# sleep3r/crispy

Measured on AMD Instinct MI355X. Metric: concurrent real-time 48 kHz streams/GPU (RNNoise), higher is better.
Workload: dtype f32; 1 GPU; Batched RNNoise: 4096 concurrent 48 kHz mono streams per GPU x 100 frames per step (BASELINE configs[1]), seeded synthetic int8 weights; streams_per_gpu=4096, output_finite=True

## Files before the change

### crispy_amd/csrc/crispy_api.cpp

```cpp
#include "../../include/crispy_hip.h"
#include "api_util.h"
#include "rn_common.h"
#include "rn_handle.h"

#include <cmath>
#include <cstdarg>
#include <cstddef>
#include <cstdio>
#include <cstdlib>
#include <cstring>
#include <new>
#include <atomic>
#include <stdexcept>
#include <string>
#include <thread>
#include <vector>

using namespace crispy;

namespace {

constexpr int kChunkFrames = 250;
#ifndef RN_SUB_FRAMES
#define RN_SUB_FRAMES 12
#endif
constexpr int kSubFrames = RN_SUB_FRAMES;
constexpr int kStagedMaxStreams = 1280;

inline const std::vector<int>& ramp_frames() {
  static const std::vector<int> ramp = [] {
    std::vector<int> r;
    if (const char* env = dev_env("CRISPY_RN_RAMP")) {
      for (const char* p = env; *p;) {
        char* end = nullptr;
        const long v = std::strtol(p, &end, 10);
        if (end == p) break;
        if (v > 0) r.push_back(v > kSubFrames ? kSubFrames : (int)v);
        p = *end ? end + 1 : end;
      }
    }
    if (r.empty()) r = {3, 4, 5, 7, 10};
    return r;
  }();
  return ramp;
}
inline int sub_frames(int index, int remaining) {
  const std::vector<int>& ramp = ramp_frames();
  const int want = index < (int)ramp.size() ? ramp[index] : kSubFrames;
  return remaining < want ? remaining : want;
}
inline int count_subs(int T) {
  int n = 0;
  for (int done = 0; done < T; ++n) done += sub_frames(n, T - done);
  return n;
}

void build_tables(RnTables* t) {
  const double pi = 3.14159265358979323846;
  for (int i = 0; i < RN_FRAME; ++i) {
    const double s = std::sin(.5 * pi * (i + .5) / RN_FRAME);
    t->half_window[i] = (float)std::sin(.5 * pi * s * s);
  }
  for (int i = 0; i < RN_NB; ++i)
    for (int j = 0; j < RN_NB; ++j) {
      double v = std::cos((i + .5) * j * pi / RN_NB);
      if (j == 0) v *= std::sqrt(.5);
      t->dct[i * RN_NB + j] = (float)v;
    }
  for (int i = 0; i < 208; ++i)
    t->tansig[i] = i <= 200 ? (float)(std::floor(std::tanh(0.04 * i) * 1e6 + 0.5) / 1e6) : 1.f;
  for (int k = 0; k < RN_WINDOW; ++k) {
    t->w960[k].x = (float)std::cos(-2.0 * pi * k / RN_WINDOW);
    t->w960[k].y = (float)std::sin(-2.0 * pi * k / RN_WINDOW);
  }
  static const int eband[RN_NB] = {0, 1, 2, 3, 4, 5, 6, 7, 8, 10, 12, 14, 16, 20, 24, 28, 34, 40, 48, 60, 78, 100};
  for (int i = 0; i < 24; ++i) t->eband[i] = i < RN_NB ? eband[i] : 100;
  for (int i = 0; i < RN_NB - 1; ++i) {
    const int bs = (eband[i + 1] - eband[i]) * 4;
    for (int j = 0; j < bs; ++j) {
      t->bin_band[eband[i] * 4 + j] = i;
      t->bin_frac[eband[i] * 4 + j] = (float)j / (float)bs;
    }
  }
  {
    int piece[64] = {0}, head[2][RN_NB];
    for (int b = 0; b < RN_NB; ++b) head[0][b] = head[1][b] = 0;
    int lane = 1;
    for (int side = 0; side < 2; ++side)
      for (int b = 0; b < RN_NB; ++b) {
        const int c0 = side == 0 ? (b > 0 ? eband[b - 1] : 0) : eband[b];
        const int c1 = side == 0 ? eband[b] : (b < RN_NB - 1 ? eband[b + 1] : eband[b]);
        const int w = (side == 0 && b == 0) ? 0 : c1 - c0;
        if (w <= 0) continue;
        const int np = (w + 5) / 6;
        if ((lane & 15) + np > 16) lane = (lane + 15) & ~15;
        if (np > 4 || lane + np > 64) std::abort();
        head[side][b] = lane;
        for (int p = 0, c = c0; p < np; ++p) {
          const int n = (w - (c - c0) + (np - p) - 1) / (np - p);
          piece[lane + p] = c | (n << 7) | (side << 10) | ((p + 1 < np ? 1 : 0) << 11) | ((p == 0 && np > 2 ? 1 : 0) << 12);
          c += n;
        }
        lane += np;
      }
    for (int l = 0; l < 64; ++l) {
      const int b = l < RN_NB ? l : 0;
      t->band_piece[l] = piece[l] | (head[0][b] << 13) | (head[1][b] << 19);
    }
  }
}

void pack_matrix(uint32_t* dst, const int8_t* src, int K, int rows, int stride) {
  const int k8n = (K + 7) / 8;
  uint16_t* h = reinterpret_cast<uint16_t*>(dst);
  for (int k8 = 0; k8 < k8n; ++k8)
    for (int r = 0; r < rows; ++r)
      for (int q = 0; q < 8; ++q) {
        const int k = 8 * k8 + q;
        const _Float16 v = (_Float16)(float)(k < K ? src[(size_t)k * stride + r] : 0);
        uint16_t bits;
        std::memcpy(&bits, &v, 2);
        h[((size_t)k8 * rows + r) * 8 + q] = bits;
      }
}

void pack_matrix8(uint32_t* dst, const int8_t* src, int K, int rows, int stride) {
  const int k16n = (K + 15) / 16;
  int8_t* b = reinterpret_cast<int8_t*>(dst);
  for (int k16 = 0; k16 < k16n; ++k16)
    for (int r = 0; r < rows; ++r)
      for (int q = 0; q < 16; ++q) {
        const int k = 16 * k16 + q;
        b[((size_t)k16 * rows + r) * 16 + q] = k < K ? src[(size_t)k * stride + r] : 0;
      }
}

void pack_bias(uint32_t* dst, const int8_t* src, int n) {
  for (int i = 0; i < n; ++i) {
    const float f = (float)src[i];
    std::memcpy(&dst[i], &f, 4);
  }
}

void pack_weights(std::vector<uint32_t>& out, const int8_t* w) {
  out.assign(RnPack8::END, 0);
  uint32_t* p = out.data();
  pack_matrix(p + 4 * RnPack::ID_W, w + RnBlob::ID_W, 42, 24, 24);
  pack_matrix(p + 4 * RnPack::VG_W, w + RnBlob::VG_W, 24, 72, 72);
  pack_matrix(p + 4 * RnPack::VG_R, w + RnBlob::VG_R, 24, 72, 72);
  pack_matrix(p + 4 * RnPack::VO_W, w + RnBlob::VO_W, 24, 1, 1);
  pack_matrix(p + 4 * RnPack::NG_W, w + RnBlob::NG_W, 90, 144, 144);
  pack_matrix(p + 4 * RnPack::NG_R, w + RnBlob::NG_R, 48, 144, 144);
  pack_matrix(p + 4 * RnPack::DG_W, w + RnBlob::DG_W, 114, 288, 288);
  pack_matrix(p + 4 * RnPack::DG_R, w + RnBlob::DG_R, 96, 288, 288);
  pack_matrix(p + 4 * RnPack::DO_W, w + RnBlob::DO_W, 96, 22, 22);
  pack_bias(p + RnPack::ID_B, w + RnBlob::ID_B, 24);
  pack_bias(p + RnPack::VG_B, w + RnBlob::VG_B, 72);
  pack_bias(p + RnPack::VO_B, w + RnBlob::VO_B, 1);
  pack_bias(p + RnPack::NG_B, w + RnBlob::NG_B, 144);
  pack_bias(p + RnPack::DG_B, w + RnBlob::DG_B, 288);
  pack_bias(p + RnPack::DO_B, w + RnBlob::DO_B, 22);
  pack_matrix8(p + 4 * RnPack8::ID_W, w + RnBlob::ID_W, 42, 24, 24);
// ... 602 lines not shown
```

### crispy_amd/csrc/rn_common.h

```cpp
#pragma once
#include <hip/hip_runtime.h>
#include <stdint.h>

namespace crispy {

constexpr int RN_FRAME = 480;
constexpr int RN_WINDOW = 960;
constexpr int RN_NFREQ = 481;
constexpr int RN_NB = 22;
constexpr int RN_NFEAT = 42;
constexpr int RN_PITCH_BUF = 1728;
constexpr int RN_HIST = 1920;
constexpr int RN_HIST_FRAMES = 4;
constexpr int RN_TAPS = 72;
constexpr int RN_WEIGHT_BYTES = 87503;
constexpr int RN_DBG_FLOATS = 4304;

struct RnTables {
  float half_window[RN_FRAME];
  float dct[RN_NB * RN_NB];
  float tansig[208];
  float2 w960[RN_WINDOW];
  float bin_frac[400];
  int bin_band[400];
  int eband[24];
  int band_piece[64];
};

struct RnBlob {
  static constexpr int ID_W = 0, ID_B = ID_W + 42 * 24;
  static constexpr int VG_W = ID_B + 24, VG_R = VG_W + 24 * 72, VG_B = VG_R + 24 * 72;
  static constexpr int VO_W = VG_B + 72, VO_B = VO_W + 24;
  static constexpr int NG_W = VO_B + 1, NG_R = NG_W + 90 * 144, NG_B = NG_R + 48 * 144;
  static constexpr int DG_W = NG_B + 144, DG_R = DG_W + 114 * 288, DG_B = DG_R + 96 * 288;
  static constexpr int DO_W = DG_B + 288, DO_B = DO_W + 96 * 22;
  static constexpr int END = DO_B + 22;
};
static_assert(RnBlob::END == RN_WEIGHT_BYTES, "blob layout");

constexpr int rn_k8(int k) { return (k + 7) / 8; }
struct RnPack {
  static constexpr int ID_W = 0;
  static constexpr int VG_W = ID_W + rn_k8(42) * 24;
  static constexpr int VG_R = VG_W + rn_k8(24) * 72;
  static constexpr int VO_W = VG_R + rn_k8(24) * 72;
  static constexpr int NG_W = VO_W + rn_k8(24) * 1;
  static constexpr int NG_R = NG_W + rn_k8(90) * 144;
  static constexpr int DG_W = NG_R + rn_k8(48) * 144;
  static constexpr int DG_R = DG_W + rn_k8(114) * 288;
  static constexpr int DO_W = DG_R + rn_k8(96) * 288;
  static constexpr int MAT_END = DO_W + rn_k8(96) * 22;
  static constexpr int ID_B = MAT_END * 4;
  static constexpr int VG_B = ID_B + 24;
  static constexpr int VO_B = VG_B + 72;
  static constexpr int NG_B = VO_B + 1;
  static constexpr int DG_B = NG_B + 144;
  static constexpr int DO_B = DG_B + 288;
  static constexpr int END = DO_B + 22;
};

constexpr int rn_k16(int k) { return (k + 15) / 16; }
struct RnPack8 {
  static constexpr int ID_W = (RnPack::END + 3) / 4;
  static constexpr int VG_W = ID_W + rn_k16(42) * 24;
  static constexpr int VG_R = VG_W + rn_k16(24) * 72;
  static constexpr int NG_W = VG_R + rn_k16(24) * 72;
  static constexpr int NG_R = NG_W + rn_k16(90) * 144;
  static constexpr int DG_W = NG_R + rn_k16(48) * 144;
  static constexpr int DG_R = DG_W + rn_k16(114) * 288;
  static constexpr int DO_W = DG_R + rn_k16(96) * 288;
  static constexpr int MAT_END = DO_W + rn_k16(96) * 22;
  static constexpr int END = MAT_END * 4;
};

struct RnArgs {
  const float* in;
  float* out;
  long stride_t, stride_b;
  int in_s16, out_s16;
// ... 226 lines not shown
```

### crispy_amd/csrc/rn_kernels.hip

```cpp
#include <type_traits>
#include "rn_common.h"
#include "rn_prio.h"
#include "rn_scale.h"
#include "rn_wave_sums.h"

namespace crispy {
namespace {

constexpr int WAVE = 64;

#ifdef RN_PROFILE
#define RN_PROF_DECL long long tprev_ = clock64(); \
  float* profp_ = (DBG && a.dbg) ? a.dbg + (long)blockIdx.x * RN_DBG_FLOATS + 3824 : nullptr; \
  rn_prof_mark(profp_, 14);
#define RN_PROF_LEAVE rn_prof_mark(profp_, 15);
#define STAMP(k) { const long long tn_ = clock64(); if (profp_ && threadIdx.x == 0) profp_[k] += (float)(tn_ - tprev_); tprev_ = tn_; }
__device__ __forceinline__ void rn_prof_mark(float* p, int k) {
  if (p && threadIdx.x == 0) {
    unsigned* u = reinterpret_cast<unsigned*>(p);
    unsigned hw, xcc;
    asm volatile("s_getreg_b32 %0, hwreg(HW_REG_HW_ID)" : "=s"(hw));
    asm volatile("s_getreg_b32 %0, hwreg(HW_REG_XCC_ID)" : "=s"(xcc));
    u[k] = (unsigned)__builtin_amdgcn_s_memrealtime();
    u[k + 2] = (unsigned)__builtin_amdgcn_s_memtime();
    u[18] = hw;
    u[19] = xcc;
  }
}
#elif defined(RN_STOP_AFTER)
#define RN_PROF_DECL
#define RN_PROF_LEAVE
#define STAMP(k) { if ((k) == RN_STOP_AFTER) { __syncthreads(); continue; } }
#else
#define RN_PROF_DECL
#define RN_PROF_LEAVE
#define STAMP(k)
#endif

__device__ __constant__ int c_second_check[16] = {0, 0, 3, 2, 3, 2, 5, 2, 3, 2, 3, 2, 5, 2, 3, 2};

__device__ __forceinline__ float2 cmul(float2 a, float2 b) {
  return make_float2(a.x * b.x - a.y * b.y, a.x * b.y + a.y * b.x);
}
__device__ __forceinline__ float2 cadd(float2 a, float2 b) { return make_float2(a.x + b.x, a.y + b.y); }
__device__ __forceinline__ float2 csub(float2 a, float2 b) { return make_float2(a.x - b.x, a.y - b.y); }
__device__ __forceinline__ float2 cconj(float2 a) { return make_float2(a.x, -a.y); }

template <int CTRL, int ROW_MASK = 0xf>
__device__ __forceinline__ float dpp_mov(float v) {
  const int iv = __float_as_int(v);
  return __int_as_float(__builtin_amdgcn_update_dpp(0, iv, CTRL, ROW_MASK, 0xf, false));
}
template <int CTRL>
__device__ __forceinline__ float dpp_add(float v) {
  float r = v + dpp_mov<CTRL>(v);
  asm volatile("" : "+v"(r));
  return r;
}
template <class V>
__device__ __forceinline__ void lane_put(V& v, V s, int l) {
  static_assert(sizeof(V) == 4, "one dword");
  asm("v_writelane_b32 %0, %1, %2" : "+v"(v) : "s"(s), "n"(l));
}
template <class T>
__device__ __forceinline__ T ld_u32(const T* __restrict__ base, unsigned idx) {
  return *reinterpret_cast<const T*>(reinterpret_cast<const char*>(base) + idx * (unsigned)sizeof(T));
}
__device__ __forceinline__ float wave_sum(float v) {
  v += dpp_mov<0xB1>(v);
  v += dpp_mov<0x4E>(v);
  v += dpp_mov<0x141>(v);
  v += dpp_mov<0x140>(v);
  v += dpp_mov<0x142, 0xa>(v);
  v += dpp_mov<0x143, 0xc>(v);
  return __int_as_float(__builtin_amdgcn_readlane(__float_as_int(v), 63));
}

template <int NW>
__device__ __forceinline__ void rn_sync() {
  if constexpr (NW == 1) {
    __syncthreads();
  } else {
    __builtin_amdgcn_fence(__ATOMIC_RELEASE, "wavefront");
    __builtin_amdgcn_s_waitcnt(0xc07f);
    __builtin_amdgcn_wave_barrier();
    __builtin_amdgcn_fence(__ATOMIC_ACQUIRE, "wavefront");
  }
}

template <int R>
__device__ __forceinline__ void butterfly(const float2 (&v)[R], float2 (&o)[R]);

template <>
__device__ __forceinline__ void butterfly<4>(const float2 (&v)[4], float2 (&o)[4]) {
  const float2 s0 = cadd(v[0], v[2]), d0 = csub(v[0], v[2]);
  const float2 s1 = cadd(v[1], v[3]), d1 = csub(v[1], v[3]);
  o[0] = cadd(s0, s1);
  o[2] = csub(s0, s1);
  o[1] = make_float2(d0.x + d1.y, d0.y - d1.x);
  o[3] = make_float2(d0.x - d1.y, d0.y + d1.x);
}
template <>
__device__ __forceinline__ void butterfly<3>(const float2 (&v)[3], float2 (&o)[3]) {
  const float2 t = cadd(v[1], v[2]), d = csub(v[1], v[2]);
  o[0] = cadd(v[0], t);
  const float2 a = make_float2(v[0].x - 0.5f * t.x, v[0].y - 0.5f * t.y);
  const float s = 0.86602540378443864676f;
  const float2 b = make_float2(s * d.x, s * d.y);
  o[1] = make_float2(a.x + b.y, a.y - b.x);
  o[2] = make_float2(a.x - b.y, a.y + b.x);
}
template <>
__device__ __forceinline__ void butterfly<5>(const float2 (&v)[5], float2 (&o)[5]) {
  const float c1 = 0.30901699437494742410f, s1 = 0.95105651629515357212f;
  const float c2 = -0.80901699437494742410f, s2 = 0.58778525229247312917f;
  const float2 t1 = cadd(v[1], v[4]), t2 = cadd(v[2], v[3]);
  const float2 t3 = csub(v[1], v[4]), t4 = csub(v[2], v[3]);
  o[0] = make_float2(v[0].x + t1.x + t2.x, v[0].y + t1.y + t2.y);
  const float2 a1 = make_float2(v[0].x + c1 * t1.x + c2 * t2.x, v[0].y + c1 * t1.y + c2 * t2.y);
  const float2 a2 = make_float2(v[0].x + c2 * t1.x + c1 * t2.x, v[0].y + c2 * t1.y + c1 * t2.y);
  const float2 b1 = make_float2(s1 * t3.x + s2 * t4.x, s1 * t3.y + s2 * t4.y);
  const float2 b2 = make_float2(s2 * t3.x - s1 * t4.x, s2 * t3.y - s1 * t4.y);
  o[1] = make_float2(a1.x + b1.y, a1.y - b1.x);
  o[4] = make_float2(a1.x - b1.y, a1.y + b1.x);
  o[2] = make_float2(a2.x + b2.y, a2.y - b2.x);
  o[3] = make_float2(a2.x - b2.y, a2.y + b2.x);
}

template <>
__device__ __forceinline__ void butterfly<8>(const float2 (&v)[8], float2 (&o)[8]) {
  const float2 ev[4] = {v[0], v[2], v[4], v[6]}, od[4] = {v[1], v[3], v[5], v[7]};
  float2 e[4], d[4];
  butterfly<4>(ev, e);
  butterfly<4>(od, d);
  const float h = 0.70710678118654752f;
  const float2 t0 = d[0];
  const float2 t1 = make_float2((d[1].x + d[1].y) * h, (d[1].y - d[1].x) * h);
  const float2 t2 = make_float2(d[2].y, -d[2].x);
  const float2 t3 = make_float2((d[3].y - d[3].x) * h, -(d[3].x + d[3].y) * h);
  o[0] = cadd(e[0], t0); o[4] = csub(e[0], t0);
  o[1] = cadd(e[1], t1); o[5] = csub(e[1], t1);
  o[2] = cadd(e[2], t2); o[6] = csub(e[2], t2);
  o[3] = cadd(e[3], t3); o[7] = csub(e[3], t3);
}

#define RN_VGPR_CAP __attribute__((amdgpu_num_vgpr(60)))
template <int R, int NS>
__device__ __forceinline__ int fft_rd(int j, int r) {
  constexpr int M = 480 / R;
  if (R == 8 && NS == 4) return (j & 3) * 120 + (j >> 2) + 15 * r;
  if (R == 3 && NS == 32) {
    const int i = j + r * M;
    return i ^ (((i >> 5) & 3) << 2);
  }
  return j + r * M;
}
template <int R, int NS>
__device__ __forceinline__ int fft_wr(int j, int r) {
  if (R == 4 && NS == 1) return r * 120 + j;
  if (R == 8 && NS == 4) {
    const int a = j >> 2, m = j & 3;
    return 32 * a + m + 4 * (r ^ (a & 3));
  }
  const int k = j % NS;
  return (j / NS) * NS * R + k + r * NS;
}
template <int NW, int R, int NS, int NSIG>
__device__ __forceinline__ void fft_pass_n(float2* const (&bufs)[NSIG], const float2* __restrict__ w960, int lane) {
  constexpr int M = 480 / R;
  constexpr int NBF = (M + WAVE - 1) / WAVE;
  float2 o[NSIG][NBF][R];
  constexpr int NTW = (NS > 1 && WAVE % NS == 0) ? 1 : NBF;
  float2 tw[NTW][R];
  if (NS > 1) {
#pragma unroll
    for (int nb = 0; nb < NTW; ++nb) {
      const unsigned k = (unsigned)min(lane + WAVE * nb, M - 1) % NS;
#pragma unroll
      for (int r = 1; r < R; ++r) tw[nb][r] = ld_u32(w960, k * (unsigned)(r * (960 / (NS * R))));
    }
  }
#pragma unroll
  for (int nb = 0; nb < NBF; ++nb) {
    const int j = lane + WAVE * nb;
    if (j < M) {
#pragma unroll
      for (int g = 0; g < NSIG; ++g) {
        float2 v[R];
#pragma unroll
        for (int r = 0; r < R; ++r) {
          float2 x = bufs[g][fft_rd<R, NS>(j, r)];
          if (NS > 1 && r > 0) x = cmul(x, tw[NTW == 1 ? 0 : nb][r]);
          v[r] = x;
        }
        butterfly<R>(v, o[g][nb]);
      }
    }
  }
  rn_sync<NW>();
#pragma unroll
  for (int nb = 0; nb < NBF; ++nb) {
    const int j = lane + WAVE * nb;
    if (j < M) {
#pragma unroll
      for (int g = 0; g < NSIG; ++g) {
#pragma unroll
        for (int r = 0; r < R; ++r) bufs[g][fft_wr<R, NS>(j, r)] = o[g][nb][r];
      }
    }
  }
  rn_sync<NW>();
}
template <int NW, int R, int NS>
__device__ __forceinline__ void fft_pass(float2* buf, const float2* __restrict__ w960, int lane) {
  float2* const bufs[1] = {buf};
  fft_pass_n<NW, R, NS, 1>(bufs, w960, lane);
}

template <int NW>
__device__ __forceinline__ void fft480(float2* buf, const float2* __restrict__ w960, int lane) {
  fft_pass<NW, 4, 1>(buf, w960, lane);
  fft_pass<NW, 8, 4>(buf, w960, lane);
  fft_pass<NW, 3, 32>(buf, w960, lane);
  fft_pass<NW, 5, 96>(buf, w960, lane);
}

template <int NW, int NSIG, class In>
__device__ __forceinline__ void fft480_from(float2* const (&bufs)[NSIG], In in, const float2* __restrict__ w960, int lane) {
  {
    float2 o[NSIG][2][4];
#pragma unroll
    for (int nb = 0; nb < 2; ++nb) {
      const int j = lane + WAVE * nb;
      if (j < 120) {
#pragma unroll
        for (int g = 0; g < NSIG; ++g) {
          float2 v[4];
#pragma unroll
          for (int r = 0; r < 4; ++r) v[r] = in(g, j, r);
          butterfly<4>(v, o[g][nb]);
        }
      }
    }
#pragma unroll
    for (int nb = 0; nb < 2; ++nb) {
      const int j = lane + WAVE * nb;
      if (j < 120) {
#pragma unroll
        for (int g = 0; g < NSIG; ++g) {
#pragma unroll
          for (int r = 0; r < 4; ++r) bufs[g][fft_wr<4, 1>(j, r)] = o[g][nb][r];
        }
      }
    }
    rn_sync<NW>();
  }
  fft_pass_n<NW, 8, 4, NSIG>(bufs, w960, lane);
  fft_pass_n<NW, 3, 32, NSIG>(bufs, w960, lane);
  fft_pass_n<NW, 5, 96, NSIG>(bufs, w960, lane);
}

template <int NW, int NSIG>
__device__ __forceinline__ void real_fwd_post(float2* const (&bufs)[NSIG], const float2* __restrict__ w960, int lane) {
  const float scale = 1.0f / 960.0f;
  float2 wk[4], wn[4];
#pragma unroll
  for (int m = 0; m < 4; ++m) {
    const unsigned k = (unsigned)min(lane + WAVE * m, 240);
    wk[m] = ld_u32(w960, k);
    wn[m] = ld_u32(w960, 480u - k);
  }
#pragma unroll
  for (int m = 0; m < 4; ++m) {
    const int k = lane + WAVE * m;
    if (k <= 240) {
#pragma unroll
      for (int g = 0; g < NSIG; ++g) {
        float2* buf = bufs[g];
        const float2 zk = buf[k];
        const float2 zn = (k == 0) ? zk : buf[480 - k];
        float2 zc = cconj(zn);
        float2 fe = make_float2(0.5f * (zk.x + zc.x), 0.5f * (zk.y + zc.y));
        float2 d = make_float2(0.5f * (zk.x - zc.x), 0.5f * (zk.y - zc.y));
        float2 t = cmul(wk[m], make_float2(d.y, -d.x));
        const float2 xk = make_float2((fe.x + t.x) * scale, (fe.y + t.y) * scale);
        zc = cconj(zk);
        fe = make_float2(0.5f * (zn.x + zc.x), 0.5f * (zn.y + zc.y));
        d = make_float2(0.5f * (zn.x - zc.x), 0.5f * (zn.y - zc.y));
        t = cmul(wn[m], make_float2(d.y, -d.x));
        const float2 xn = make_float2((fe.x + t.x) * scale, (fe.y + t.y) * scale);
        buf[k] = xk;
        buf[480 - k] = xn;
      }
    }
  }
  rn_sync<NW>();
}

template <int NW>
__device__ __forceinline__ void real_inv_pre(float2* buf, const float2* __restrict__ w960, int lane) {
  float2 wk[4], wn[4];
#pragma unroll
  for (int m = 0; m < 4; ++m) {
    const unsigned k = (unsigned)min(lane + WAVE * m, 240);
    wk[m] = ld_u32(w960, k);
    wn[m] = ld_u32(w960, 480u - k);
  }
#pragma unroll
  for (int m = 0; m < 4; ++m) {
    const int k = lane + WAVE * m;
    if (k <= 240) {
      const float2 a = buf[k];
      const float2 bn = buf[480 - k];
      float2 b = cconj(bn);
      float2 fe = cadd(a, b);
      float2 fo = cmul(csub(a, b), cconj(wk[m]));
      const float2 zk = make_float2(fe.x - fo.y, -(fe.y + fo.x));
      b = cconj(a);
      fe = cadd(bn, b);
      fo = cmul(csub(bn, b), cconj(wn[m]));
      const float2 zn = make_float2(fe.x - fo.y, -(fe.y + fo.x));
      buf[k] = zk;
      if (k > 0) buf[480 - k] = zn;
    }
  }
  rn_sync<NW>();
}

struct BandEdges {
  int piece;
};

__device__ __forceinline__ float band_sum(const float* part_lo, const float* part_hi, const BandEdges& be, int lane) {
  int bd = be.piece;
  asm volatile("" : "+v"(bd));
  const int n = (bd >> 7) & 7;
  const float* p = ((bd >> 10) & 1 ? part_lo : part_hi) + (bd & 127);
  float v[6];
#pragma unroll
  for (int k = 0; k < 6; ++k) v[k] = p[k];
  float s = 0.f;
#pragma unroll
  for (int k = 0; k < 6; ++k) s += k < n ? v[k] : 0.f;
  {
    const float t1 = dpp_mov<0x101>(s);
    s += (bd >> 11) & 1 ? t1 : 0.f;
    const float t2 = dpp_mov<0x102>(s);
    s += (bd >> 12) & 1 ? t2 : 0.f;
  }
  const float rise = __int_as_float(__builtin_amdgcn_ds_bpermute(((bd >> 13) & 63) << 2, __float_as_int(s)));
  const float fall = __int_as_float(__builtin_amdgcn_ds_bpermute(((bd >> 19) & 63) << 2, __float_as_int(s)));
  float tot = rise + fall;
  if (lane == 0 || lane == RN_NB - 1) tot *= 2.f;
  return tot;
}

template <int NW, bool CORR, bool XE = false>
__device__ __forceinline__ void band_pairs(const float2* S, const float2* Xc, float* part, float* Eout, float* Cout,
                                           float* Xout, float2* park, const RnTables* __restrict__ tab,
                                           const BandEdges& be, int lane) {
  float clo[4], chi[4];
  float xlo[4], xhi[4];
  float2 fr[4];
#pragma unroll
  for (int m = 0; m < 4; ++m) fr[m] = ld_u32(reinterpret_cast<const float2*>(tab->bin_frac), (unsigned)min(lane + WAVE * m, 199));
  float4 svq[4];
#pragma unroll
  for (int m = 0; m < 4; ++m) svq[m] = *reinterpret_cast<const float4*>(S + 2 * min(lane + WAVE * m, 199));
#pragma unroll
  for (int m = 0; m < 4; ++m) {
    const int pidx = lane + WAVE * m;
    clo[m] = 0.f; chi[m] = 0.f;
    if (pidx < 200) {
      const float2 f = fr[m];
      const float4 sv = svq[m];
      float e0 = sv.x * sv.x; e0 += sv.y * sv.y;
      float e1 = sv.z * sv.z; e1 += sv.w * sv.w;
      float lo = (1.f - f.x) * e0 + (1.f - f.y) * e1;
      float hi = f.x * e0 + f.y * e1;
      lo = dpp_add<0xB1>(lo);
      hi = dpp_add<0xB1>(hi);
      if ((lane & 1) == 0) { part[pidx >> 1] = lo; part[100 + (pidx >> 1)] = hi; }
      if (CORR) {
        const float4 xv = *reinterpret_cast<const float4*>(Xc + 2 * pidx);
        float c0 = xv.x * sv.x; c0 += xv.y * sv.y;
        float c1 = xv.z * sv.z; c1 += xv.w * sv.w;
        float l2 = (1.f - f.x) * c0 + (1.f - f.y) * c1;
        float h2 = f.x * c0 + f.y * c1;
        clo[m] = dpp_add<0xB1>(l2);
        chi[m] = dpp_add<0xB1>(h2);
        if (XE) {
          float x0, x1, l3, h3;
          if (m == 0) {
            x0 = fmaf(xv.y, xv.y, xv.x * xv.x);
            x1 = fmaf(xv.w, xv.w, xv.z * xv.z);
            l3 = fmaf(1.f - f.y, x1, (1.f - f.x) * x0);
            h3 = fmaf(f.y, x1, f.x * x0);
          } else {
            x0 = fmaf(xv.x, xv.x, xv.y * xv.y);
            x1 = fmaf(xv.z, xv.z, xv.w * xv.w);
            l3 = fmaf(1.f - f.x, x0, (1.f - f.y) * x1);
// ... 232 lines not shown
                                            float* state, float* zbuf, signed char* st_img, int toff,
                                            const TansigTab& tansig, int lane) {
  constexpr int ROWS = 3 * N;
  constexpr int MK16 = (M + 15) / 16, NK16 = (N + 15) / 16;
  constexpr int NRZ = (2 * N + WAVE - 1) / WAVE, NRC = (N + WAVE - 1) / WAVE;
  const float S = 1.f / 256.f;
  const RnScale sst = image_i8<NK16 * 16>(st_img, lane, [&](int i) { return i < N ? state[min(i, N - 1)] : 0.f; });
  rn_sync<NW>();
  {
    int rows[NRZ];
    float acc[NRZ];
#pragma unroll
    for (int r = 0; r < NRZ; ++r) {
      rows[r] = min(lane + WAVE * r, 2 * N - 1);
      acc[r] = ld_u32(bias, (unsigned)rows[r]);
    }
    dotn_i<MK16, NK16, ROWS, NRZ, rn_chains(NW)>(rs, w_off, u_off, rows, in_img, st_img, toff, sin, sst.dn, acc);
#pragma unroll
    for (int r = 0; r < NRZ; ++r) {
      const int row = lane + WAVE * r;
      const float s = sigmoid_approx(S * acc[r], tansig);
      if (row < 2 * N) {
        if (row < N) zbuf[row] = s;
        else digits_store(st_img, row - N, state[row - N] * s, sst.up);
      }
    }
  }
  rn_sync<NW>();
  {
    int rows[NRC];
    float acc[NRC];
#pragma unroll
    for (int r = 0; r < NRC; ++r) {
      rows[r] = 2 * N + min(lane + WAVE * r, N - 1);
      acc[r] = ld_u32(bias, (unsigned)rows[r]);
    }
    dotn_i<MK16, NK16, ROWS, NRC, rn_chains(NW)>(rs, w_off, u_off, rows, in_img, st_img, toff, sin, sst.dn, acc);
#pragma unroll
    for (int r = 0; r < NRC; ++r) {
      const int i = lane + WAVE * r;
      if (i < N) {
        float c = S * acc[r];
        c = c < 0.f ? 0.f : c;
        const float z = zbuf[i];
        state[i] = z * state[i] + (1.f - z) * c;
      }
    }
  }
  rn_sync<NW>();
}

struct alignas(16) RnSlot {
  float2 A[482];
  float2 Bb[482];
  float U[200];
  float Ex[24], Ep[24], Exp[24];
  int pitch_index;
  float pitch_gain;
  int silence;
  int pad;
};
template <int NW> struct RnLdsT;
template <> struct alignas(16) RnLdsT<1> {
  RnSlot s[1];
  float ceps[8 * 22];
  float rnn_state[168];
};
template <> struct alignas(16) RnLdsT<3> {
  RnSlot s[2];
  float2 pa[482];
  float2 pb[482];
  float ceps[8 * 22];
  float rnn_state[168];
  int pitch_index[2];
  float pitch_gain[2];
};
static_assert(sizeof(RnLdsT<1>) <= 10240, "16 workgroups per CU need <= 10 KB of LDS each");
static_assert(6 * sizeof(RnLdsT<3>) <= 160 * 1024, "six stage-pipelined streams per CU");

constexpr int U_G = 0, U_R = 24, U_VAD = 46, U_LY = 48;
constexpr int PL_FEAT = 800, PL_Z = 842, PL_DENSE = 938, PL_A_FREE = 800, PL_U_FREE = 48;

__device__ __forceinline__ float lane_up(float v, int lane4, int off) {
  return __int_as_float(__builtin_amdgcn_ds_bpermute(lane4 + 4 * (WAVE - off), __float_as_int(v)));
}

struct Cand {
  float num, den;
  int idx;
};
__device__ __forceinline__ bool cand_better(const Cand& a, const Cand& b) {
  const float l = a.num * b.den, r = b.num * a.den;
  const bool gt = l > r, ngt = !(r > l), lt = a.idx < b.idx;
  return gt | (ngt & lt);
}
__device__ __forceinline__ Cand cand_pick(bool take_a, const Cand& a, const Cand& b) {
  return Cand{take_a ? a.num : b.num, take_a ? a.den : b.den, take_a ? a.idx : b.idx};
}
template <int OFF>
__device__ __forceinline__ int lane_xor(int v) {
  return __builtin_amdgcn_ds_swizzle(v, (OFF << 10) | 0x1f);
}
template <int OFF>
__device__ __forceinline__ Cand cand_xor(const Cand& c) {
  return Cand{__int_as_float(lane_xor<OFF>(__float_as_int(c.num))), __int_as_float(lane_xor<OFF>(__float_as_int(c.den))),
              lane_xor<OFF>(c.idx)};
}
__device__ __forceinline__ Cand wave_best(Cand c, int half_addr) {
  {
    const Cand o = {__int_as_float(__builtin_amdgcn_ds_bpermute(half_addr, __float_as_int(c.num))),
                    __int_as_float(__builtin_amdgcn_ds_bpermute(half_addr, __float_as_int(c.den))),
                    __builtin_amdgcn_ds_bpermute(half_addr, c.idx)};
    c = cand_pick(cand_better(o, c), o, c);
  }
  { const Cand o = cand_xor<16>(c); c = cand_pick(cand_better(o, c), o, c); }
  { const Cand o = cand_xor<8>(c); c = cand_pick(cand_better(o, c), o, c); }
  { const Cand o = cand_xor<4>(c); c = cand_pick(cand_better(o, c), o, c); }
  { const Cand o = cand_xor<2>(c); c = cand_pick(cand_better(o, c), o, c); }
  { const Cand o = cand_xor<1>(c); c = cand_pick(cand_better(o, c), o, c); }
  c.num = __int_as_float(__builtin_amdgcn_readlane(__float_as_int(c.num), 0));
  c.den = __int_as_float(__builtin_amdgcn_readlane(__float_as_int(c.den), 0));
  c.idx = __builtin_amdgcn_readlane(c.idx, 0);
  return c;
}

typedef float rn_f2 __attribute__((ext_vector_type(2)));
__device__ __forceinline__ void lag_window(const float* xr, int lane, float (&xv)[8]) {
#pragma unroll
  for (int m = 0; m < 7; ++m) xv[m] = xr[WAVE * m];
  xv[7] = 0.f;
  if (lane < 32) xv[7] = xr[WAVE * 7];
// ... 457 lines not shown
          const float g1 = xyk / sqrtf(1.f + xx * yyk);
          float cont;
          if (abs(T1 - prev_period) <= 1) cont = last_gain;
          else if (abs(T1 - prev_period) <= 2 && 5 * k * k < T0) cont = .5f * last_gain;
          else cont = 0.f;
          float thresh = fmaxf(.3f, .7f * g0 - cont);
          if (T1 < 90) thresh = fmaxf(.4f, .85f * g0 - cont);
          else if (T1 < 60) thresh = fmaxf(.5f, .9f * g0 - cont);
          const unsigned long long pass = __ballot(lane < 14 && T1 >= 30 && g1 > thresh);
          if (pass != 0ull) {
            const int w = 63 - __builtin_clzll(pass);
            best_xy = __int_as_float(__builtin_amdgcn_readlane(__float_as_int(xyk), w));
            best_yy = __int_as_float(__builtin_amdgcn_readlane(__float_as_int(yyk), w));
            T = __builtin_amdgcn_readlane(T1, w);
            g = __int_as_float(__builtin_amdgcn_readlane(__float_as_int(g1), w));
          }
        }
        best_xy = fmaxf(0.f, best_xy);
        float pgv = (best_yy <= best_xy) ? 1.f : best_xy / (best_yy + 1.f);
        float xc3[3];
        {
          const float* yr[3] = {x - (T - 1) + lane, x - T + lane, x - (T + 1) + lane};
          float sb[3];
          lag_dots<3, false>(xwin, yr, lane, xc3, sb);
        }
        int offset = 0;
        if ((xc3[2] - xc3[0]) > .7f * (xc3[1] - xc3[0])) offset = 1;
        else if ((xc3[0] - xc3[2]) > .7f * (xc3[1] - xc3[2])) offset = -1;
        if (pgv > g) pgv = g;
        pitch_index = 2 * T + offset;
        if (pitch_index < 60) pitch_index = 60;
        pitch_gain = pgv;
        last_period = pitch_index;
        last_gain = pgv;
      }
      rn_sync<NW>();
      STAMP(4)
      if constexpr (NW > 1) {
        if (lane == 0) { L.pitch_index[t & 1] = pitch_index; L.pitch_gain[t & 1] = pitch_gain; }
      }
    }
    if (own_b) {
      if constexpr (NW > 1) {
        pitch_index = __builtin_amdgcn_readfirstlane(L.pitch_index[t & 1]);
        pitch_gain = L.pitch_gain[t & 1];
      }
      lane = lane0;
      asm volatile("" : "+v"(lane));
      RN_LANE_RANGE(5);

      {
        const float* pp = pb + (768 - pitch_index);
        float2* const xp[2] = {SL.A, SL.Bb};
        fft480_from<NW, 2>(xp, [&](int g, int j, int r) {
          const int n = j + 120 * r;
          const float w0 = r < 2 ? hw[2 * n] : hw[959 - 2 * n];
          const float w1 = r < 2 ? hw[2 * n + 1] : hw[958 - 2 * n];
          if (g == 0) {
            const float2 v = *reinterpret_cast<const float2*>(xw + 2 * n);
            return make_float2(v.x * w0, v.y * w1);
          }
          return make_float2(pp[2 * n] * w0, pp[2 * n + 1] * w1);
        }, w960, lane);
        real_fwd_post<NW, 2>(xp, w960, lane);
      }
      STAMP(5)
      band_pairs<NW, true, true>(SL.Bb, SL.A, SL.U, SL.Ep, SL.Exp, SL.Ex, nullptr, tab, be, lane);
      if (DBG && a.dbg && t == a.T - 1) {
        float* D = a.dbg + (long)b * RN_DBG_FLOATS;
        const float* Pf = reinterpret_cast<const float*>(SL.Bb);
        for (int i = lane; i < 962; i += WAVE) { D[0 + i] = Xf[i]; D[1856 + i] = Pf[i]; }
        if (lane < RN_NB) D[962 + lane] = SL.Ex[lane];
      }
      rn_sync<NW>();
      STAMP(6)
      lane = lane0;
      asm volatile("" : "+v"(lane));
      RN_LANE_RANGE(7);

      float dctc[RN_NB];
      {
        const float* __restrict__ dcol = tab->dct + min(lane, RN_NB - 1);
  #pragma unroll
        for (int j = 0; j < RN_NB; ++j) dctc[j] = dcol[j * RN_NB];
      }
      if (lane < RN_NB) {
        SL.Exp[lane] = SL.Exp[lane] / sqrtf(.001f + SL.Ex[lane] * SL.Ep[lane]);
        SL.U[U_LY + lane] = log10f(1e-2f + SL.Ex[lane]);
      }
      rn_sync<NW>();
      if (DBG && a.dbg && t == a.T - 1 && lane < RN_NB) {
        float* D = a.dbg + (long)b * RN_DBG_FLOATS;
        D[2818 + lane] = SL.Ep[lane];
        D[2840 + lane] = SL.Exp[lane];
      }
      const float dct_norm = 0.30151134457776363f;
      float E = 0.f;
      float se = 0.f, sl = 0.f;
      {
        float logMax = -2.f, follow = -2.f;
  #pragma unroll
        for (int i = 0; i < RN_NB; ++i) {
          float ly = SL.U[U_LY + i];
          ly = fmaxf(logMax - 7.f, fmaxf(follow - 1.5f, ly));
          logMax = fmaxf(logMax, ly);
          follow = fmaxf(follow - 1.5f, ly);
          E += SL.Ex[i];
          sl = fmaf(ly, dctc[i], sl);
          se = fmaf(SL.Exp[i], dctc[i], se);
          if (i % 4 == 3) {
            asm volatile("" : "+v"(sl), "+v"(se), "+v"(E), "+v"(logMax), "+v"(follow));
            __builtin_amdgcn_sched_barrier(0);
          }
        }
      }
      {
// ... 180 lines not shown
          lastg = gg;
        }
        rn_sync<NW>();
        float nq[4][2], gq[4][2];
        float4 xq[4];
  #pragma unroll
        for (int m = 0; m < 4; ++m) {
          nq[m][0] = SL.U[U_R + bq[m]]; nq[m][1] = SL.U[U_R + bq[m] + 1];
          gq[m][0] = SL.U[U_G + bq[m]]; gq[m][1] = SL.U[U_G + bq[m] + 1];
          xq[m] = *reinterpret_cast<const float4*>(SL.A + 2 * min(lane + WAVE * m, 199));
        }
  #pragma unroll
        for (int m = 0; m < 4; ++m) {
          const int pidx = lane + WAVE * m;
          if (pidx < 200) {
            const float n0 = nq[m][0], n1 = nq[m][1];
            const float g0 = gq[m][0], g1 = gq[m][1];
            const float nf0 = (1.f - fq[m].x) * n0 + fq[m].x * n1, nf1 = (1.f - fq[m].y) * n0 + fq[m].y * n1;
            const float gf0 = (1.f - fq[m].x) * g0 + fq[m].x * g1, gf1 = (1.f - fq[m].y) * g0 + fq[m].y * g1;
            float4 x = xq[m];
            x.x *= nf0; x.y *= nf0; x.z *= nf1; x.w *= nf1;
            x.x *= gf0; x.y *= gf0; x.z *= gf1; x.w *= gf1;
            *reinterpret_cast<float4*>(SL.A + 2 * pidx) = x;
          }
        }
        for (int i = 400 + lane; i < RN_NFREQ; i += WAVE) SL.A[i] = make_float2(0.f, 0.f);
        rn_sync<NW>();
      }
      STAMP(11)

      if (DBG && a.taps) {
        float* tp = a.taps + ((long)t * a.B + b) * RN_TAPS;
        if (lane < RN_NFEAT) tp[lane] = Rb[KB_FEAT + lane];
        if (lane < RN_NB) tp[42 + lane] = SL.U[U_G + lane];
        if (lane == 0) {
          tp[64] = (float)pitch_index;
          tp[65] = pitch_gain;
          tp[66] = vad_prob;
          tp[67] = silence ? 1.f : 0.f;
          tp[68] = tp[69] = tp[70] = tp[71] = 0.f;
        }
      }
      if (a.vad && lane == 0) a.vad[(long)t * a.B + b] = vad_prob;
      if (DBG && a.dbg && t == a.T - 1) {
        float* D = a.dbg + (long)b * RN_DBG_FLOATS;
        for (int i = lane; i < 962; i += WAVE) D[2862 + i] = Xf[i];
      }
      rn_sync<NW>();

      lane = lane0;
      asm volatile("" : "+v"(lane));
      RN_LANE_RANGE(3);
      real_inv_pre<NW>(SL.A, w960, lane);
      fft480<NW>(SL.A, w960, lane);
      STAMP(12)
      {
        float* o = a.out + (long)t * a.stride_t + (long)b * a.stride_b;
        float2 hwa[4], hwb[4];
  #pragma unroll
        for (int m = 0; m < 4; ++m) {
          const unsigned n = (unsigned)min(lane + WAVE * m, 239);
          hwa[m] = ld_u32(reinterpret_cast<const float2*>(hw), n);
          hwb[m] = ld_u32(reinterpret_cast<const float2*>(hw), 239u - n);
        }
  #pragma unroll
        for (int m = 0; m < 4; ++m) {
          const int n = lane + WAVE * m;
          if (n < 240) {
            const float2 z = SL.A[n];
            const float2 z2 = SL.A[240 + n];
            const int i0 = 2 * n;
            float2 ov;
            ov.x = fmaf(z.x, hwa[m].x, synth[m].x);
            ov.y = fmaf(-z.y, hwa[m].y, synth[m].y);
            if (a.out_s16) {
              const float q0 = truncf(fminf(fmaxf(ov.x * (1.f / 32768.f), -1.f), 1.f) * 32767.f);
              const float q1 = truncf(fminf(fmaxf(ov.y * (1.f / 32768.f), -1.f), 1.f) * 32767.f);
              const unsigned pk = ((unsigned)(int)q0 & 0xffffu) | ((unsigned)(int)q1 << 16);
              __builtin_nontemporal_store(pk, reinterpret_cast<unsigned*>(reinterpret_cast<int16_t*>(a.out) + (long)t * a.stride_t + (long)b * a.stride_b + i0));
            } else {
              __builtin_nontemporal_store(ov.x, o + i0); __builtin_nontemporal_store(ov.y, o + i0 + 1);
            }
            synth[m].x = z2.x * hwb[m].y;
            synth[m].y = -z2.y * hwb[m].x;
          }
        }
      }
      rn_sync<NW>();
      STAMP(13)
    }
    }
    if constexpr (NW > 1) __syncthreads();
  }
  RN_PROF_LEAVE

  if (own_c) {
#pragma unroll
    for (int m = 0; m < 4; ++m) {
      const int n = lane + WAVE * m;
      if (n < 240) *reinterpret_cast<float2*>(synth_g + 2 * n) = synth[m];
    }
    for (int i = lane; i < 168; i += WAVE) a.rnn[(long)b * 168 + i] = L.rnn_state[i];
    if (lane < RN_NB) a.lastg[(long)b * RN_NB + lane] = lastg;
  }
  if (own_b) {
    for (int i = lane; i < 176; i += WAVE) a.ceps[(long)b * 176 + i] = L.ceps[i];
    if (lane == 0) a.memid[b] = memid;
// ... 47 lines not shown
```

### crispy_amd/csrc/rn_wave_sums.h

```cpp
#pragma once
#include <hip/hip_runtime.h>

namespace crispy {

template <int CTRL, int ROW_MASK = 0xf>
__device__ __forceinline__ float ws_dpp(float v) {
  const int iv = __float_as_int(v);
  return __int_as_float(__builtin_amdgcn_update_dpp(0, iv, CTRL, ROW_MASK, 0xf, false));
}
__device__ __forceinline__ void ws_swap32(float& a, float& b) {
  const auto r = __builtin_amdgcn_permlane32_swap(__float_as_uint(a), __float_as_uint(b), false, false);
  a = __uint_as_float(r[0]);
  b = __uint_as_float(r[1]);
}
__device__ __forceinline__ void ws_swap16(float& a, float& b) {
  const auto r = __builtin_amdgcn_permlane16_swap(__float_as_uint(a), __float_as_uint(b), false, false);
  a = __uint_as_float(r[0]);
  b = __uint_as_float(r[1]);
}
__device__ __forceinline__ float ws_rows(float q) {
  q += ws_dpp<0xB1>(q);
  q += ws_dpp<0x4E>(q);
  q += ws_dpp<0x141>(q);
  q += ws_dpp<0x140>(q);
  return q;
}
__device__ __forceinline__ float ws_lane(float v, int l) {
  return __int_as_float(__builtin_amdgcn_readlane(__float_as_int(v), l));
}
__device__ __forceinline__ void wave_sum4(float& a, float& b, float& c, float& d) {
  ws_swap32(a, b);
  float ab = a + b;
  ws_swap32(c, d);
  float cd = c + d;
  ws_swap16(ab, cd);
  const float q = ws_rows(ab + cd);
  a = ws_lane(q, 0);
  c = ws_lane(q, 16);
  b = ws_lane(q, 32);
  d = ws_lane(q, 48);
}
__device__ __forceinline__ void wave_sum2(float& a, float& b) {
  ws_swap32(a, b);
  float q = ws_rows(a + b);
  q += ws_dpp<0x142, 0xa>(q);
  a = ws_lane(q, 31);
  b = ws_lane(q, 63);
}
__device__ __forceinline__ float wave_sum1(float v) {
  v = ws_rows(v);
  v += ws_dpp<0x142, 0xa>(v);
  v += ws_dpp<0x143, 0xc>(v);
  return ws_lane(v, 63);
}
template <int N>
__device__ __forceinline__ void wave_sums(float (&v)[N]) {
  int i = 0;
#pragma unroll
  for (; i + 4 <= N; i += 4) wave_sum4(v[i], v[i + 1], v[i + 2], v[i + 3]);
  if (N - i == 3) {
    float z = 0.f;
    wave_sum4(v[i], v[i + 1], v[i + 2], z);
  } else if (N - i == 2) {
    wave_sum2(v[i], v[i + 1]);
  } else if (N - i == 1) {
    v[i] = wave_sum1(v[i]);
  }
}

}
```

Baseline: 800,800 concurrent real-time 48 kHz streams (whole job).

## Use per-pass twiddle row tables, joint half-wave FFT trip, and DPP micro-optimizations

Precomputes per-pass FFT twiddle rows (radix 8, 3, 5) so each lane loads its twiddles as float4 rows instead of gathering scattered w960 entries. For the two-signal FFT it also merges the half-filled final trip of both signals into one wave-wide trip. Further changes fuse the DPP row-broadcast reductions into inline asm adds, make the band-sum masking branchless, reorder the LDS slot layout so lag windows sit on 256-byte steps, and use unsigned-offset loads for the window. Together these aim to cut global gather loads, idle lanes and instruction count. The catch is extra table memory, hand-written asm with manual s_nop hazards, and band_piece flag bits whose meaning changed.

Result: faster. 819,300 concurrent real-time 48 kHz streams (whole job), median of 6 (+2.3%).

```diff
diff --git a/crispy_amd/csrc/crispy_api.cpp b/crispy_amd/csrc/crispy_api.cpp
--- a/crispy_amd/csrc/crispy_api.cpp
+++ b/crispy_amd/csrc/crispy_api.cpp
@@ -1,6 +1,8 @@
 #include "../../include/crispy_hip.h"
 #include "api_util.h"
+#include "rn_band_piece.h"
 #include "rn_common.h"
+#include "rn_twiddle_rows.h"
 #include "rn_handle.h"
 
 #include <cmath>
@@ -73,7 +75,9 @@
     t->w960[k].x = (float)std::cos(-2.0 * pi * k / RN_WINDOW);
     t->w960[k].y = (float)std::sin(-2.0 * pi * k / RN_WINDOW);
   }
-  static const int eband[RN_NB] = {0, 1, 2, 3, 4, 5, 6, 7, 8, 10, 12, 14, 16, 20, 24, 28, 34, 40, 48, 60, 78, 100};
+  rn_build_twiddle_rows(t->w960, t->tw8, t->tw3, t->tw5);
+  static_assert(RN_BANDS == RN_NB, "rn_band_piece.h");
+  const int (&eband)[RN_NB] = kRnEband;
   for (int i = 0; i < 24; ++i) t->eband[i] = i < RN_NB ? eband[i] : 100;
   for (int i = 0; i < RN_NB - 1; ++i) {
     const int bs = (eband[i + 1] - eband[i]) * 4;
@@ -82,32 +86,7 @@
       t->bin_frac[eband[i] * 4 + j] = (float)j / (float)bs;
     }
   }
-  {
-    int piece[64] = {0}, head[2][RN_NB];
-    for (int b = 0; b < RN_NB; ++b) head[0][b] = head[1][b] = 0;
-    int lane = 1;
-    for (int side = 0; side < 2; ++side)
-      for (int b = 0; b < RN_NB; ++b) {
-        const int c0 = side == 0 ? (b > 0 ? eband[b - 1] : 0) : eband[b];
-        const int c1 = side == 0 ? eband[b] : (b < RN_NB - 1 ? eband[b + 1] : eband[b]);
-        const int w = (side == 0 && b == 0) ? 0 : c1 - c0;
-        if (w <= 0) continue;
-        const int np = (w + 5) / 6;
-        if ((lane & 15) + np > 16) lane = (lane + 15) & ~15;
-        if (np > 4 || lane + np > 64) std::abort();
-        head[side][b] = lane;
-        for (int p = 0, c = c0; p < np; ++p) {
-          const int n = (w - (c - c0) + (np - p) - 1) / (np - p);
-          piece[lane + p] = c | (n << 7) | (side << 10) | ((p + 1 < np ? 1 : 0) << 11) | ((p == 0 && np > 2 ? 1 : 0) << 12);
-          c += n;
-        }
-        lane += np;
-      }
-    for (int l = 0; l < 64; ++l) {
-      const int b = l < RN_NB ? l : 0;
-      t->band_piece[l] = piece[l] | (head[0][b] << 13) | (head[1][b] << 19);
-    }
-  }
+  if (!rn_build_band_piece(t->band_piece)) std::abort();
 }
 
 void pack_matrix(uint32_t* dst, const int8_t* src, int K, int rows, int stride) {
diff --git a/crispy_amd/csrc/rn_band_piece.h b/crispy_amd/csrc/rn_band_piece.h
--- /dev/null
+++ b/crispy_amd/csrc/rn_band_piece.h
@@ -0,0 +1,36 @@
+#pragma once
+
+namespace crispy {
+
+constexpr int RN_BANDS = 22;
+constexpr int kRnEband[RN_BANDS] = {0, 1, 2, 3, 4, 5, 6, 7, 8, 10, 12, 14, 16, 20, 24, 28, 34, 40, 48, 60, 78, 100};
+
+inline bool rn_build_band_piece(int (&out)[64]) {
+  int piece[64] = {0}, head[2][RN_BANDS];
+  for (int b = 0; b < RN_BANDS; ++b) head[0][b] = head[1][b] = 0;
+  int lane = 1;
+  for (int side = 0; side < 2; ++side)
+    for (int b = 0; b < RN_BANDS; ++b) {
+      const int c0 = side == 0 ? (b > 0 ? kRnEband[b - 1] : 0) : kRnEband[b];
+      const int c1 = side == 0 ? kRnEband[b] : (b < RN_BANDS - 1 ? kRnEband[b + 1] : kRnEband[b]);
+      const int w = (side == 0 && b == 0) ? 0 : c1 - c0;
+      if (w <= 0) continue;
+      const int np = (w + 5) / 6;
+      if ((lane & 15) + np > 16) lane = (lane + 15) & ~15;
+      if (np > 4 || lane + np > 64) return false;
+      head[side][b] = lane;
+      for (int p = 0, c = c0; p < np; ++p) {
+        const int n = (w - (c - c0) + (np - p) - 1) / (np - p);
+        piece[lane + p] = c | (n << 7) | (side << 10) | ((p >= 1 ? 1 : 0) << 11) | ((p == 2 ? 1 : 0) << 12);
+        c += n;
+      }
+      lane += np;
+    }
+  for (int l = 0; l < 64; ++l) {
+    const int b = l < RN_BANDS ? l : 0;
+    out[l] = piece[l] | (head[0][b] << 13) | (head[1][b] << 19);
+  }
+  return true;
+}
+
+}
diff --git a/crispy_amd/csrc/rn_common.h b/crispy_amd/csrc/rn_common.h
--- a/crispy_amd/csrc/rn_common.h
+++ b/crispy_amd/csrc/rn_common.h
@@ -25,6 +25,9 @@
   int bin_band[400];
   int eband[24];
   int band_piece[64];
+  alignas(16) float2 tw8[4][8];
+  alignas(16) float2 tw3[32][2];
+  alignas(16) float2 tw5[96][4];
 };
 
 struct RnBlob {
diff --git a/crispy_amd/csrc/rn_kernels.hip b/crispy_amd/csrc/rn_kernels.hip
--- a/crispy_amd/csrc/rn_kernels.hip
+++ b/crispy_amd/csrc/rn_kernels.hip
@@ -57,6 +57,12 @@
   asm volatile("" : "+v"(r));
   return r;
 }
+template <int CTRL>
+__device__ __forceinline__ float dpp_add_of(float v, float u) {
+  float r = v + dpp_mov<CTRL>(u);
+  asm volatile("" : "+v"(r));
+  return r;
+}
 template <class V>
 __device__ __forceinline__ void lane_put(V& v, V s, int l) {
   static_assert(sizeof(V) == 4, "one dword");
@@ -71,8 +77,7 @@
   v += dpp_mov<0x4E>(v);
   v += dpp_mov<0x141>(v);
   v += dpp_mov<0x140>(v);
-  v += dpp_mov<0x142, 0xa>(v);
-  v += dpp_mov<0x143, 0xc>(v);
+  v = ws_join_rows(v);
   return __int_as_float(__builtin_amdgcn_readlane(__float_as_int(v), 63));
 }
 
@@ -166,22 +171,38 @@
   return (j / NS) * NS * R + k + r * NS;
 }
 template <int NW, int R, int NS, int NSIG>
-__device__ __forceinline__ void fft_pass_n(float2* const (&bufs)[NSIG], const float2* __restrict__ w960, int lane) {
+__device__ __forceinline__ void fft_pass_n(float2* const (&bufs)[NSIG], const RnTables* __restrict__ tab, int lane) {
   constexpr int M = 480 / R;
   constexpr int NBF = (M + WAVE - 1) / WAVE;
-  float2 o[NSIG][NBF][R];
+  constexpr bool JOINT = NSIG == 2 && NBF > 1 && M % WAVE == WAVE / 2;
+  constexpr int NFULL = JOINT ? NBF - 1 : NBF;
+  const int jm = M - WAVE / 2 + (lane & (WAVE / 2 - 1));
+  float2 o[NSIG][NFULL][R];
+  [[maybe_unused]] float2 om[R];
   constexpr int NTW = (NS > 1 && WAVE % NS == 0) ? 1 : NBF;
+  static_assert(!JOINT || NTW == NBF || (M - WAVE / 2) % NS == 0, "the joint trip shares the twiddles of the full trips");
   float2 tw[NTW][R];
   if (NS > 1) {
+    static_assert(NS == 1 || (R == 8 && NS == 4) || (R == 3 && NS == 32) || (R == 5 && NS == 96), "a row table per pass");
+    constexpr int RQ = R == 8 ? 4 : (R - 1) / 2;
+    typedef const __attribute__((address_space(1))) float4* GRowPtr;
+    GRowPtr rowg = (GRowPtr)reinterpret_cast<const float4*>(R == 8 ? &tab->tw8[0][0] : (R == 3 ? &tab->tw3[0][0] : &tab->tw5[0][0]));
+    asm volatile("" : "+s"(rowg));
+    const float4* rows = (const float4*)rowg;
 #pragma unroll
     for (int nb = 0; nb < NTW; ++nb) {
-      const unsigned k = (unsigned)min(lane + WAVE * nb, M - 1) % NS;
-#pragma unroll
-      for (int r = 1; r < R; ++r) tw[nb][r] = ld_u32(w960, k * (unsigned)(r * (960 / (NS * R))));
-    }
-  }
-#pragma unroll
-  for (int nb = 0; nb < NBF; ++nb) {
+      const unsigned k = (unsigned)(JOINT && nb == NBF - 1 ? jm : min(lane + WAVE * nb, M - 1)) % NS;
+#pragma unroll
+      for (int q = 0; q < RQ; ++q) {
+        const float4 t = ld_u32(rows, k * (unsigned)RQ + q);
+        const int r0 = R == 8 ? 2 * q : 2 * q + 1;
+        if (r0 > 0) tw[nb][r0] = make_float2(t.x, t.y);
+        tw[nb][r0 + 1] = make_float2(t.z, t.w);
+      }
+    }
+  }
+#pragma unroll
+  for (int nb = 0; nb < NFULL; ++nb) {
     const int j = lane + WAVE * nb;
     if (j < M) {
 #pragma unroll
@@ -197,9 +218,20 @@
       }
     }
   }
+  float2* const bm = bufs[JOINT && lane >= WAVE / 2 ? 1 : 0];
+  if constexpr (JOINT) {
+    float2 v[R];
+#pragma unroll
+    for (int r = 0; r < R; ++r) {
+      float2 x = bm[fft_rd<R, NS>(jm, r)];
+      if (NS > 1 && r > 0) x = cmul(x, tw[NTW == 1 ? 0 : NBF - 1][r]);
+      v[r] = x;
+    }
+    butterfly<R>(v, om);
+  }
   rn_sync<NW>();
 #pragma unroll
-  for (int nb = 0; nb < NBF; ++nb) {
+  for (int nb = 0; nb < NFULL; ++nb) {
     const int j = lane + WAVE * nb;
     if (j < M) {
 #pragma unroll
@@ -209,24 +241,28 @@
       }
     }
   }
+  if constexpr (JOINT) {
+#pragma unroll
+    for (int r = 0; r < R; ++r) bm[fft_wr<R, NS>(jm, r)] = om[r];
+  }
   rn_sync<NW>();
 }
 template <int NW, int R, int NS>
-__device__ __forceinline__ void fft_pass(float2* buf, const float2* __restrict__ w960, int lane) {
+__device__ __forceinline__ void fft_pass(float2* buf, const RnTables* __restrict__ tab, int lane) {
   float2* const bufs[1] = {buf};
-  fft_pass_n<NW, R, NS, 1>(bufs, w960, lane);
+  fft_pass_n<NW, R, NS, 1>(bufs, tab, lane);
 }
 
 template <int NW>
-__device__ __forceinline__ void fft480(float2* buf, const float2* __restrict__ w960, int lane) {
-  fft_pass<NW, 4, 1>(buf, w960, lane);
-  fft_pass<NW, 8, 4>(buf, w960, lane);
-  fft_pass<NW, 3, 32>(buf, w960, lane);
-  fft_pass<NW, 5, 96>(buf, w960, lane);
+__device__ __forceinline__ void fft480(float2* buf, const RnTables* __restrict__ tab, int lane) {
+  fft_pass<NW, 4, 1>(buf, tab, lane);
+  fft_pass<NW, 8, 4>(buf, tab, lane);
+  fft_pass<NW, 3, 32>(buf, tab, lane);
+  fft_pass<NW, 5, 96>(buf, tab, lane);
 }
 
 template <int NW, int NSIG, class In>
-__device__ __forceinline__ void fft480_from(float2* const (&bufs)[NSIG], In in, const float2* __restrict__ w960, int lane) {
+__device__ __forceinline__ void fft480_from(float2* const (&bufs)[NSIG], In in, const RnTables* __restrict__ tab, int lane) {
   {
     float2 o[NSIG][2][4];
 #pragma unroll
@@ -255,9 +291,9 @@
     }
     rn_sync<NW>();
   }
-  fft_pass_n<NW, 8, 4, NSIG>(bufs, w960, lane);
-  fft_pass_n<NW, 3, 32, NSIG>(bufs, w960, lane);
-  fft_pass_n<NW, 5, 96, NSIG>(bufs, w960, lane);
+  fft_pass_n<NW, 8, 4, NSIG>(bufs, tab, lane);
+  fft_pass_n<NW, 3, 32, NSIG>(bufs, tab, lane);
+  fft_pass_n<NW, 5, 96, NSIG>(bufs, tab, lane);
 }
 
 template <int NW, int NSIG>
@@ -343,10 +379,9 @@
 #pragma unroll
   for (int k = 0; k < 6; ++k) s += k < n ? v[k] : 0.f;
   {
-    const float t1 = dpp_mov<0x101>(s);
-    s += (bd >> 11) & 1 ? t1 : 0.f;
-    const float t2 = dpp_mov<0x102>(s);
-    s += (bd >> 12) & 1 ? t2 : 0.f;
+    const int g1 = (bd << 20) >> 31, g2 = (bd << 19) >> 31;
+    s = dpp_add_of<0x101>(s, __int_as_float(__float_as_int(s) & g1));
+    s = dpp_add_of<0x102>(s, __int_as_float(__float_as_int(s) & g2));
   }
   const float rise = __int_as_float(__builtin_amdgcn_ds_bpermute(((bd >> 13) & 63) << 2, __float_as_int(s)));
   const float fall = __int_as_float(__builtin_amdgcn_ds_bpermute(((bd >> 19) & 63) << 2, __float_as_int(s)));
@@ -685,14 +720,16 @@
 
 struct alignas(16) RnSlot {
   float2 A[482];
-  float2 Bb[482];
-  float U[200];
-  float Ex[24], Ep[24], Exp[24];
+  float Ex[24], Ep[24];
   int pitch_index;
   float pitch_gain;
   int silence;
-  int pad;
+  int pad[9];
+  float2 Bb[482];
+  float U[200];
+  float Exp[24];
 };
+static_assert(offsetof(RnSlot, Bb) % 256 == 0, "lag windows in 256-byte steps");
 template <int NW> struct RnLdsT;
 template <> struct alignas(16) RnLdsT<1> {
   RnSlot s[1];
@@ -702,6 +739,7 @@
 template <> struct alignas(16) RnLdsT<3> {
   RnSlot s[2];
   float2 pa[482];
+  float pad[52];
   float2 pb[482];
   float ceps[8 * 22];
   float rnn_state[168];
@@ -710,6 +748,7 @@
 };
 static_assert(sizeof(RnLdsT<1>) <= 10240, "16 workgroups per CU need <= 10 KB of LDS each");
 static_assert(6 * sizeof(RnLdsT<3>) <= 160 * 1024, "six stage-pipelined streams per CU");
+static_assert(offsetof(RnLdsT<3>, pb) % 256 == 0, "lag windows in 256-byte steps");
 
 constexpr int U_G = 0, U_R = 24, U_VAD = 46, U_LY = 48;
 constexpr int PL_FEAT = 800, PL_Z = 842, PL_DENSE = 938, PL_A_FREE = 800, PL_U_FREE = 48;
@@ -1273,16 +1312,18 @@
       {
         const float* pp = pb + (768 - pitch_index);
         float2* const xp[2] = {SL.A, SL.Bb};
+        const float2* hw2 = reinterpret_cast<const float2*>(hw);
         fft480_from<NW, 2>(xp, [&](int g, int j, int r) {
-          const int n = j + 120 * r;
-          const float w0 = r < 2 ? hw[2 * n] : hw[959 - 2 * n];
-          const float w1 = r < 2 ? hw[2 * n + 1] : hw[958 - 2 * n];
+          const unsigned n = (unsigned)j + 120u * r;
+          float w0, w1;
+          if (r < 2) { const float2 w = ld_u32(hw2, n); w0 = w.x; w1 = w.y; }
+          else { const float2 w = ld_u32(hw2, 479u - n); w0 = w.y; w1 = w.x; }
           if (g == 0) {
-            const float2 v = *reinterpret_cast<const float2*>(xw + 2 * n);
+            const float2 v = ld_u32(reinterpret_cast<const float2*>(xw), n);
             return make_float2(v.x * w0, v.y * w1);
           }
-          return make_float2(pp[2 * n] * w0, pp[2 * n + 1] * w1);
-        }, w960, lane);
+          return make_float2(ld_u32(pp, 2u * n) * w0, ld_u32(pp, 2u * n + 1u) * w1);
+        }, tab, lane);
         real_fwd_post<NW, 2>(xp, w960, lane);
       }
       STAMP(5)
@@ -1569,7 +1610,7 @@
       asm volatile("" : "+v"(lane));
       RN_LANE_RANGE(3);
       real_inv_pre<NW>(SL.A, w960, lane);
-      fft480<NW>(SL.A, w960, lane);
+      fft480<NW>(SL.A, tab, lane);
       STAMP(12)
       {
         float* o = a.out + (long)t * a.stride_t + (long)b * a.stride_b;
diff --git a/crispy_amd/csrc/rn_twiddle_rows.h b/crispy_amd/csrc/rn_twiddle_rows.h
--- /dev/null
+++ b/crispy_amd/csrc/rn_twiddle_rows.h
@@ -0,0 +1,17 @@
+#pragma once
+
+namespace crispy {
+
+constexpr int rn_twiddle_step(int R, int NS) { return 960 / (NS * R); }
+
+template <class C>
+inline void rn_build_twiddle_rows(const C (&w960)[960], C (&tw8)[4][8], C (&tw3)[32][2], C (&tw5)[96][4]) {
+  for (int k = 0; k < 4; ++k)
+    for (int r = 0; r < 8; ++r) tw8[k][r] = w960[k * r * rn_twiddle_step(8, 4)];
+  for (int k = 0; k < 32; ++k)
+    for (int r = 1; r < 3; ++r) tw3[k][r - 1] = w960[k * r * rn_twiddle_step(3, 32)];
+  for (int k = 0; k < 96; ++k)
+    for (int r = 1; r < 5; ++r) tw5[k][r - 1] = w960[k * r * rn_twiddle_step(5, 96)];
+}
+
+}
diff --git a/crispy_amd/csrc/rn_wave_sums.h b/crispy_amd/csrc/rn_wave_sums.h
--- a/crispy_amd/csrc/rn_wave_sums.h
+++ b/crispy_amd/csrc/rn_wave_sums.h
@@ -7,6 +7,15 @@
 __device__ __forceinline__ float ws_dpp(float v) {
   const int iv = __float_as_int(v);
   return __int_as_float(__builtin_amdgcn_update_dpp(0, iv, CTRL, ROW_MASK, 0xf, false));
+}
+__device__ __forceinline__ float ws_join_rows(float v) {
+  asm("s_nop 4\n\tv_add_f32_dpp %0, %0, %0 row_bcast:15 row_mask:0xa bank_mask:0xf\n\t"
+      "s_nop 1\n\tv_add_f32_dpp %0, %0, %0 row_bcast:31 row_mask:0xc bank_mask:0xf\n\ts_nop 0" : "+v"(v));
+  return v;
+}
+__device__ __forceinline__ float ws_join_row_pairs(float v) {
+  asm("s_nop 4\n\tv_add_f32_dpp %0, %0, %0 row_bcast:15 row_mask:0xa bank_mask:0xf\n\ts_nop 0" : "+v"(v));
+  return v;
 }
 __device__ __forceinline__ void ws_swap32(float& a, float& b) {
   const auto r = __builtin_amdgcn_permlane32_swap(__float_as_uint(a), __float_as_uint(b), false, false);
@@ -42,16 +51,12 @@
 }
 __device__ __forceinline__ void wave_sum2(float& a, float& b) {
   ws_swap32(a, b);
-  float q = ws_rows(a + b);
-  q += ws_dpp<0x142, 0xa>(q);
+  const float q = ws_join_row_pairs(ws_rows(a + b));
   a = ws_lane(q, 31);
   b = ws_lane(q, 63);
 }
 __device__ __forceinline__ float wave_sum1(float v) {
-  v = ws_rows(v);
-  v += ws_dpp<0x142, 0xa>(v);
-  v += ws_dpp<0x143, 0xc>(v);
-  return ws_lane(v, 63);
+  return ws_lane(ws_join_rows(ws_rows(v)), 63);
 }
 template <int N>
 __device__ __forceinline__ void wave_sums(float (&v)[N]) {
```
